# marcin119a/vae-los-angeles

Hardware: AMD Instinct MI355X
Metric: training samples/sec, MultiModalVAE batch 65536 (higher is better)
Workload: dtype bf16

## Files before the change

### include/mmvae_hip.h

```cpp
#ifndef MMVAE_HIP_H
#define MMVAE_HIP_H
#include <stdint.h>

#ifdef __cplusplus
extern "C" {
#endif

#define MMVAE_OK 0
#define MMVAE_ERR_ARG (-1)
#define MMVAE_ERR_DTYPE (-2)

enum { MMVAE_F32 = 0, MMVAE_BF16 = 1 };
enum { MMVAE_PREC_F32 = 0, MMVAE_PREC_BF16 = 1 };
enum { MMVAE_PRO_NONE = 0, MMVAE_PRO_BN_RELU_DROP = 1, MMVAE_PRO_BN_BWD_APPLY = 2 };
enum { MMVAE_EPI_STORE = 0, MMVAE_EPI_RELU_MASK = 1, MMVAE_EPI_BN_BWD = 2, MMVAE_EPI_LOSS_MSE = 3, MMVAE_EPI_LOSS_BCE_LOGIT = 4 };
enum { MMVAE_ACT_NONE = 0, MMVAE_ACT_RELU = 1, MMVAE_ACT_SIGMOID = 2 };

#define MMVAE_TILE 128

int mmvae_abi_version(void);
int mmvae_set_tuning(int32_t key, int32_t value);

typedef struct {
    const float* src; void* dst;
// ... 101 lines not shown
    const void* w; int64_t ldw; const float* bias;
} mmvae_latent_enc;
typedef struct {
    int32_t prec, B, L, n_mod;
    mmvae_latent_enc enc_a, enc_b;
    const float* table; const int64_t* site; int32_t S;
    const float* eps;
    float* mu; float* logvar;
    void* z; int64_t ldz;
    const void* w_stem; int64_t ldw_stem; const float* bias_stem; int32_t N_stem;
    void* h0; int64_t ldh0;
} mmvae_latent_fwd_args;
int mmvae_latent_fwd(const mmvae_latent_fwd_args* args, void* stream);

typedef struct {
    int32_t prec, B, S, L, hidden;
    const void* h0; int64_t ldh0;
    const void* w; int64_t ldw; const void* wt; int64_t ldwt; const float* bias;
    const int64_t* site; const float* class_weights;
    const float* mu; const float* logvar;
    float beta, gamma; const float* beta_gamma_dev;
    double* sums;
    float* g_c; int64_t ld_gc;
    void* d0; int64_t ldd0;
    float* g_mu; float* g_lv;
} mmvae_class_tail_args;
int mmvae_class_tail(const mmvae_class_tail_args* args, void* stream);
int mmvae_class_tail_fits(int32_t prec, int32_t S, int32_t hidden, int32_t L, int64_t ldh0, int64_t ldd0);

typedef struct {
// ... 99 lines not shown
```

### vae-los-angeles_amd/csrc/common.h

```cpp
#pragma once
#include <hip/hip_runtime.h>
#include <stdint.h>
#include "mmvae_hip.h"

namespace mm {

typedef __bf16 bf16;
typedef __attribute__((ext_vector_type(8))) __bf16 bf16x8;
typedef __attribute__((ext_vector_type(4))) __bf16 bf16x4;
typedef __attribute__((ext_vector_type(2))) __bf16 bf16x2;
typedef __attribute__((ext_vector_type(4))) float f32x4;
typedef __attribute__((ext_vector_type(2))) float f32x2;
typedef __attribute__((ext_vector_type(4))) short s16x4;

constexpr int WAVE = 64;
constexpr int TILE = 128;
constexpr int NTHREADS = 256;
constexpr int ROW_BYTES = 128;
constexpr int NUM_CU = 256;

template <typename CT> struct Mma;

template <> struct Mma<bf16> {
    static constexpr int EPC = 8;
// ... 127 lines not shown
#endif


struct Tuning {
    int nt_wide_min_m = NUM_CU * 128;
    int nt2_on = 1;
    long split_bytes = 1L << 32;
    long block_bytes = 1L << 31;
    int tn_wide_on = 1;
    int bnbwd_stream = 1;
    int relu_stream = 1;
    int ntp_on = 1;
    int ntp_min_m = 16384;
    int latent_on = 1;
    int class_tail_on = 1;
};
inline Tuning g_tuning;

constexpr int NOT_TAKEN = 1 << 30;

template <auto Kernel, typename... Args>
inline int launch_lds(dim3 grid, dim3 block, int lds, hipStream_t st, const Args&... args) {
    static bool attr_done = false;
    if (!attr_done) {
        hipError_t e = hipFuncSetAttribute((const void*)Kernel, hipFuncAttributeMaxDynamicSharedMemorySize, lds);
        if (e != hipSuccess) return (int)e;
        attr_done = true;
    }
    hipLaunchKernelGGL(Kernel, grid, block, lds, st, args...);
    return (int)hipGetLastError();
// ... 49 lines not shown
```

### vae-los-angeles_amd/csrc/elementwise.hip

```cpp
#include <vector>
#include "common.h"
#include "mmvae_hip.h"
#include "fuse_math.h"
#include "loss_terms.h"

namespace mm {

__global__ __launch_bounds__(256) void prep_weights_kernel(const mmvae_prep_item* __restrict__ items) {
    const mmvae_prep_item it = items[blockIdx.y];
    __shared__ float tile[32][33];
    const int tx = threadIdx.x & 31, ty = threadIdx.x >> 5;
    const int tiles_c = (it.dst_cols + 31) / 32, tiles_r = (it.dst_rows + 31) / 32;
    auto put = [&](int r, int c, float v) {
        if (it.dst_dtype == MMVAE_BF16) ((bf16*)it.dst)[(long)r * it.dst_ld + c] = (bf16)v;
        else ((float*)it.dst)[(long)r * it.dst_ld + c] = v;
    };
    for (int t = blockIdx.x; t < tiles_r * tiles_c; t += gridDim.x) {
        const int tr = t / tiles_c, tc = t - tr * tiles_c;
        if (it.transpose) {
#pragma unroll
            for (int k = 0; k < 4; ++k) {
                const int sr = tc * 32 + ty + 8 * k, sc = tr * 32 + tx;
                tile[ty + 8 * k][tx] = (sr < it.src_rows && sc < it.src_cols) ? it.src[(long)sr * it.src_ld + sc] : 0.f;
            }
// ... 227 lines not shown
            const long i = min(i0 + (long)u * blockDim.x, iend - 1);
            const int b = (int)(i / a.L), l = (int)(i - (long)b * a.L);
            bb[u] = b; ll[u] = l;
            dz[u] = a.dz[(long)b * a.lddz + l];
            if (a.dz2) dz[u] += a.dz2[(long)b * a.lddz + l];
            if (a.dz3) dz[u] += a.dz3[(long)b * a.lddz + l];
            gm[u] = a.g_mu ? a.g_mu[i] : 0.f; gl[u] = a.g_lv ? a.g_lv[i] : 0.f;
            ep[u] = a.eps[i]; lv[u] = a.logvar[i];
            sidx[u] = a.d_table ? a.site[b] : 0;
            if (sidx[u] < 0 || sidx[u] >= a.S) sidx[u] = -1;
        }
#pragma unroll
        for (int u = 0; u < U; ++u) {
            if (i0 + (long)u * blockDim.x >= iend) break;
            const int b = bb[u], l = ll[u];
            float dmu = gm[u] + dz[u];
            float dlv = gl[u] + dz[u] * ep[u] * expf(0.5f * lv[u]) * 0.5f;
            if (a.n_mod > 1) { dmu *= inv_n; dlv *= inv_n; }
            a.d_heads[(long)b * a.ld_heads + l] = dmu;
            a.d_heads[(long)b * a.ld_heads + a.L + l] = dlv;
            if (a.d_heads_lp) {
                bf16* lp = (bf16*)a.d_heads_lp + (long)b * a.ld_heads_lp;
                lp[l] = (bf16)dmu; lp[a.L + l] = (bf16)dlv;
                if (l == 0) for (int e = 2 * a.L; e < a.ld_heads_lp; ++e) lp[e] = (bf16)0.f;
            }
            if (a.d_table && sidx[u] >= 0) {
                const long sx = sidx[u];
                if (use_lds) { atomicAdd(&sT[sx * L2 + l], dmu); atomicAdd(&sT[sx * L2 + a.L + l], dlv); }
                else { unsafeAtomicAdd(&dtab[sx * L2 + l], dmu); unsafeAtomicAdd(&dtab[sx * L2 + a.L + l], dlv); }
            }
        }
    }
    if (use_lds && a.d_table) {
// ... 750 lines not shown
```

### vae-los-angeles_amd/csrc/fuse_math.h

```cpp
#pragma once
#include "common.h"

namespace mm {

__device__ __forceinline__ float fuse_reparam_elem(float& mu, float& lv, int n_mod, float inv_n, float eps) {
    if (n_mod > 1) { mu *= inv_n; lv *= inv_n; }
    return mu + eps * expf(0.5f * lv);
}

}
```

### vae-los-angeles_amd/csrc/gemm_nt.hip

```cpp
#include "common.h"
#include "mmvae_hip.h"
#include "gemm_src.h"
#include "gemm_nt_epi.h"
#include "gemm_nt2.h"

namespace mm {

STAMP_BUFFER(nt)

__device__ __forceinline__ int swz(int row, int chunk) { return row * ROW_BYTES + ((chunk ^ (row & 7)) << 4); }

template <int WN> struct NtLds {
    static constexpr int BUF = (TILE + 64 * WN) * ROW_BYTES;
    static constexpr int STAGE = 2 * BUF;
    static constexpr int ECOL = STAGE + 4096 + 4 * 64 * WN * 4;
    static constexpr int TOTAL = ECOL + 8 * 64 * WN * 4;
};

template <typename CT, typename Src, typename Epi, int WN>
__global__ __launch_bounds__(128 * WN, 2)
void gemm_nt_kernel(Src src, const CT* __restrict__ W, long ldw, int M, int N, int K, int gx, int gy, Epi epi)
{
    constexpr int EPC = Mma<CT>::EPC;
    constexpr int BK = ROW_BYTES / (int)sizeof(CT);
// ... 293 lines not shown
    switch (key) {
    case 0: t.nt_wide_min_m = value; return 0;
    case 2: t.nt2_on = value; return 0;
    case 3:
        if (value != 0 && (value < 17 || value > 32)) return MMVAE_ERR_ARG;
        t.split_bytes = value ? 1L << value : mm::Tuning{}.split_bytes;
        t.block_bytes = t.split_bytes / 2;
        return 0;
    case 4: t.tn_wide_on = value; return 0;
    case 6: t.bnbwd_stream = value; return 0;
    case 7: t.relu_stream = value; return 0;
    case 8: t.ntp_on = value; return 0;
    case 9: t.ntp_min_m = value; return 0;
    case 10: t.latent_on = value; return 0;
    case 12: t.class_tail_on = value; return 0;
    }
    return MMVAE_ERR_ARG;
}

extern "C" int mmvae_gemm_nt(const mmvae_gemm_nt_args* a, void* stream) {
    if (!a || !a->a || !a->w || (!a->c && !(a->epilogue == MMVAE_EPI_BN_BWD && a->bn_phase == 0))) return MMVAE_ERR_ARG;
    if (a->M <= 0 || a->N <= 0 || a->K <= 0) return MMVAE_ERR_ARG;
    if (a->ldw % 64 || ((uintptr_t)a->w & 15)) return MMVAE_ERR_ARG;
    const long lim = 1L << 32;
    if (((long)a->N + 256) * a->ldw * 4 >= lim) return MMVAE_ERR_ARG;
    const long a_row = (long)a->lda * (a->a_dtype == MMVAE_BF16 ? 2 : 4);
    long row_bytes = a_row > (long)a->ld_pro_mask ? a_row : (long)a->ld_pro_mask;
    if (!mm::bn_fin_ok(a)) return MMVAE_ERR_ARG;
    if (mm::needs_row_blocks(a->M, row_bytes)) {
        if (a->pro_finalize || a->pro_out) return MMVAE_ERR_ARG;
// ... 23 lines not shown
```

### vae-los-angeles_amd/csrc/gemm_nt2.h

```cpp
#pragma once
#include "common.h"
#include "gemm_nt_epi.h"

namespace mm {

template <int WN> struct Nt2Lds {
    static constexpr int A_BYTES = TILE * ROW_BYTES;
    static constexpr int W_BYTES = 64 * WN * ROW_BYTES;
    static constexpr int SLOT = A_BYTES + W_BYTES;
    static constexpr int RING = 2 * SLOT;
    static constexpr int RED = RING;
    static constexpr int ECOL = RED + 4 * 64 * WN * 4;
    static constexpr int TOTAL = ECOL + 8 * 64 * WN * 4;
};

STAMP_BUFFER(nt2)

typedef __attribute__((address_space(3))) void lds_void;
typedef __attribute__((address_space(1))) const void gbl_void;

template <typename Epi, int WN>
__device__ __forceinline__ void nt2_loss_epilogue(unsigned char* smem, const float* ecol, float* red, f32x4 (&acc)[4][4], const Epi& epi,
                                                  int row0, int col0, int M, int N, int tid, int lane, int wr, int wc)
{
// ... 147 lines not shown
    __syncthreads();
    const int ccols = (int)min((long)((N + 7) & ~7), epi.ldc);
    const unsigned char* src = smem + r0 * 512 + ((c ^ (r0 & 7)) << 4);
    float sc[4], sh[4], mu[4], rs[4], s1[4] = {0.f, 0.f, 0.f, 0.f}, s2[4] = {0.f, 0.f, 0.f, 0.f};
#pragma unroll
    for (int e = 0; e < 4; ++e) { sc[e] = ecol[4 * c + e]; sh[e] = ecol[BN + 4 * c + e]; mu[e] = ecol[2 * BN + 4 * c + e]; rs[e] = ecol[3 * BN + 4 * c + e]; }
#pragma unroll
    for (int i = 0; i < 16; ++i) {
        const int grow = row0 + r0 + 8 * i;
        const f32x4 z = *(const f32x4*)(src + i * 8 * 512);
        bf16x4 o;
#pragma unroll
        for (int e = 0; e < 4; ++e) {
            const bool ok = grow < M && colg + e < N;
            const float y = (float)yv[i][e];
            const float keep = ((mv[i] >> (8 * e)) & 0xffu) ? epi.inv_keep : 0.f;
            const float d = (ok && y * sc[e] + sh[e] > 0.f) ? z[e] * (has_mask ? keep : 1.f) : 0.f;
            const float xh = (y - mu[e]) * rs[e];
            s1[e] += d; s2[e] += d * xh;
            o[e] = (bf16)d;
        }
        if (grow < M && colg < ccols) *(bf16x4*)(C + (long)grow * epi.ldc + colg) = o;
    }
    __syncthreads();
    float* part = (float*)smem;
#pragma unroll
    for (int e = 0; e < 4; ++e) { part[(r0 * 2 + 0) * BN + 4 * c + e] = s1[e]; part[(r0 * 2 + 1) * BN + 4 * c + e] = s2[e]; }
    __syncthreads();
    if (tid < 2 * BN) {
        const int which = tid >> 7, col = tid & (BN - 1);
        float v = 0.f;
#pragma unroll
        for (int g = 0; g < 8; ++g) v += part[(g * 2 + which) * BN + col];
// ... 145 lines not shown
```

### vae-los-angeles_amd/mmvae/_lib.py

```python
import ctypes as C
import os

_HERE = os.path.dirname(os.path.abspath(__file__))
LIB_PATH = os.environ.get("MMVAE_LIB_PATH") or os.path.join(_HERE, "libmmvae_hip.so")
ABI_VERSION = 20

F32, BF16 = 0, 1
PREC_F32, PREC_BF16 = 0, 1
PRO_NONE, PRO_BN_RELU_DROP, PRO_BN_BWD_APPLY = 0, 1, 2
TABLE_COPIES = 8
EPI_STORE, EPI_RELU_MASK, EPI_BN_BWD, EPI_LOSS_MSE, EPI_LOSS_BCE_LOGIT = 0, 1, 2, 3, 4
ACT_NONE, ACT_RELU, ACT_SIGMOID = 0, 1, 2
TILE = 128
TN_GROUP_MAX = 8
KNN_MAXK = 64
SIL_MAXC = 64
PCA_MAXK = 64
CTR_COPIES = 16384

i32, i64, f32, vp = C.c_int32, C.c_int64, C.c_float, C.c_void_p


class PrepItem(C.Structure):
    _fields_ = [("src", vp), ("dst", vp), ("src_rows", i32), ("src_cols", i32), ("src_ld", i64),
# ... 55 lines not shown

class LatentEnc(C.Structure):
    _fields_ = [("y", vp), ("ldy", i64), ("K", i32), ("scale", vp), ("shift", vp),
                ("mask", vp), ("ld_mask", i64), ("inv_keep", f32), ("finalize", vp),
                ("w", vp), ("ldw", i64), ("bias", vp)]


class LatentFwdArgs(C.Structure):
    _fields_ = [("prec", i32), ("B", i32), ("L", i32), ("n_mod", i32),
                ("enc_a", LatentEnc), ("enc_b", LatentEnc),
                ("table", vp), ("site", vp), ("S", i32),
                ("eps", vp), ("mu", vp), ("logvar", vp),
                ("z", vp), ("ldz", i64),
                ("w_stem", vp), ("ldw_stem", i64), ("bias_stem", vp), ("N_stem", i32),
                ("h0", vp), ("ldh0", i64)]


class ClassTailArgs(C.Structure):
    _fields_ = [("prec", i32), ("B", i32), ("S", i32), ("L", i32), ("hidden", i32),
                ("h0", vp), ("ldh0", i64),
                ("w", vp), ("ldw", i64), ("wt", vp), ("ldwt", i64), ("bias", vp),
                ("site", vp), ("class_weights", vp),
                ("mu", vp), ("logvar", vp),
                ("beta", f32), ("gamma", f32), ("beta_gamma_dev", vp),
                ("sums", vp),
                ("g_c", vp), ("ld_gc", i64),
                ("d0", vp), ("ldd0", i64),
                ("g_mu", vp), ("g_lv", vp)]


# ... 62 lines not shown
    "mmvae_set_tuning": [i32, i32],
    "mmvae_prep_weights": [vp, i32, vp],
    "mmvae_gemm_nt": [C.POINTER(GemmNtArgs), vp],
    "mmvae_gemm_tn": [C.POINTER(GemmTnArgs), vp],
    "mmvae_gemm_tn_group": [vp, i32, vp],
    "mmvae_bn_finalize": [C.POINTER(BnFinalizeArgs), vp],
    "mmvae_bn_eval_coeffs": [i32, vp, vp, vp, vp, f32, vp, vp, vp, vp, vp],
    "mmvae_bn_bwd_finalize": [C.POINTER(BnBwdFinalizeArgs), vp],
    "mmvae_bn_bwd_apply": [i32, i32, i32, vp, i64, vp, i64, vp, vp, vp, vp],
    "mmvae_bn_bwd_finalize_apply": [i32, i32, i32, vp, i64, vp, i64, vp, vp, vp, vp, vp, vp, vp, i32, vp],
    "mmvae_embed_table_fwd": [i32, i32, i32, vp, vp, vp, vp, vp, vp, vp],
    "mmvae_embed_table_bwd": [i32, i32, i32, vp, vp, vp, vp, i32, vp, vp, vp, vp, vp, vp],
    "mmvae_fuse_reparam_fwd": [C.POINTER(FuseFwdArgs), vp],
    "mmvae_fuse_reparam_bwd": [C.POINTER(FuseBwdArgs), vp],
    "mmvae_latent_fwd": [C.POINTER(LatentFwdArgs), vp],
    "mmvae_class_tail": [C.POINTER(ClassTailArgs), vp],
    "mmvae_class_tail_fits": [i32, i32, i32, i32, i64, i64],
    "mmvae_vae_loss": [C.POINTER(LossArgs), vp],
    "mmvae_loss_finalize": [vp, f32, f32, vp, vp, vp],
    "mmvae_recon_metrics": [C.POINTER(MetricsArgs), vp],
    "mmvae_knn_search": [C.POINTER(KnnArgs), vp],
    "mmvae_knn_work_bytes": [i32, i32, i32, C.POINTER(i64)],
    "mmvae_knn_splits": [i32, i32, C.POINTER(i32), C.POINTER(i32)],
    "mmvae_knn_mean_rows": [vp, i64, vp, i32, i64, vp, i64, i32, i32, i32, i32, vp],
    "mmvae_silhouette_samples": [C.POINTER(SilhouetteArgs), vp],
    "mmvae_silhouette_work_bytes": [i32, i32, i32, C.POINTER(i64)],
    "mmvae_silhouette_splits": [i32, i32, i32, C.POINTER(i32)],
    "mmvae_pca_scatter": [C.POINTER(PcaScatterArgs), vp],
    "mmvae_pca_scatter_splits": [i32, i32, i32, C.POINTER(i32)],
    "mmvae_pca_scatter_work_bytes": [i32, i32, i32, C.POINTER(i64)],
# ... 51 lines not shown
```

### vae-los-angeles_amd/mmvae/engine.py

```python
import os
from dataclasses import dataclass
from typing import NamedTuple, Optional

import torch

from . import ops
from . import _lib as L_
from .ops import (PREC_BF16, PREC_F32, ACT_NONE, ACT_RELU, ACT_SIGMOID, EPI_RELU_MASK, EPI_BN_BWD, DROP_P,
                  ceil_to, act_dtype, Prologue, BnBwdEpilogue, BnBwdFinalize, BnBwdApply)

_PRECISIONS = {"bf16": PREC_BF16, "fp32": PREC_F32, "f32": PREC_F32}
_default_precision = _PRECISIONS[os.environ.get("MMVAE_PRECISION", "bf16").lower()]
_TINY_DW_MAX = 16384


def set_default_precision(name):
    global _default_precision
    _default_precision = _PRECISIONS[name.lower()]


def default_precision():
    return _default_precision


# ... 254 lines not shown
            else:
                ops.gemm_nt(prec, h, pl.w, N, K, y, bias=pl.bias, prologue=pro, tag=f"{self.name}.L{len(layers)}.fwd")
                ops.bn_eval_coeffs(bn.weight, bn.bias, bn.running_mean, bn.running_var, st.scale, st.shift, bn.eps, st.mean, st.rstd)
                new_pro = Prologue(st.scale, st.shift, None, 1.0)
            layers.append(LayerSave(h, pro, y, st, new_pro) if h_act is None else LayerSave(h_act, None, y, st, new_pro))
            h, pro = y, new_pro
        owed = ops.LatentEncoder(h, pro, fin, self.pl_heads)
        return (self.run_heads(prec, owed) if heads else owed), layers

    def run_heads(self, prec, owed):
        heads = torch.empty(owed.y.shape[0], 2 * self.latent, dtype=torch.float32, device=owed.y.device)
        self._consume(prec, owed.y, owed.prologue, owed.fin, 2 * self.latent, self.pl_heads.K, heads, self.pl_heads.bias, self.pl_heads.w,
                      f"{self.name}.heads.fwd")
        return heads

    def backward(self, prec, layers, d_heads, grads, tn=ops.gemm_tn, stats_bufs=None, train=True, d_heads_lp=None):
        B, dev = d_heads.shape[0], d_heads.device
        adt = act_dtype(prec)
        L2 = 2 * self.latent
        Kl = self.pl_heads.K
        gw = grads[self.fc_mu.weight]
        gb = grads[self.fc_mu.bias]
        tn(prec, d_heads, layers[-1].y, _span(gw, L2 * Kl).view(L2, Kl), _span(gb, L2), L2, Kl, q_prologue=layers[-1].y_prologue, tag=f"{self.name}.heads.dW")
        src, src_wt, src_n, src_k = (d_heads_lp if d_heads_lp is not None else d_heads), self.pl_heads.wt, Kl, L2
        for i in reversed(range(len(self.linears))):
            lin, bn, pl = self.linears[i], self.bns[i], self.pl[i]
            sv = layers[i]
            y = sv.y
            st = sv.bn
            N, K = pl.N, pl.K
            bnargs = BnBwdEpilogue(st.scale, st.shift, st.mean, st.rstd, sv.y_prologue.mask, sv.y_prologue.inv_keep)
            stats = stats_bufs[i] if stats_bufs is not None else torch.zeros(2, N, dtype=torch.float64, device=dev)
            coef = torch.empty(3, N, dtype=torch.float32, device=dev)
            d = torch.empty(B, ceil_to(N, 8), dtype=adt, device=dev)
            ops.gemm_nt(prec, src, src_wt, src_n, src_k, d, epilogue=EPI_BN_BWD, h=y, bn=bnargs, bn_phase=2, stats=stats, tag=f"{self.name}.L{i}.dX")
            fin = BnBwdFinalize(stats, bn.weight, grads[bn.weight], grads[bn.bias], not train)
            if i == 0 and K <= 4096:
                if prec == PREC_BF16 and B >= 8192 and N >= 128 and K >= 256:
                    try:
                        tn(prec, d, sv.q, grads[lin.weight], grads[lin.bias], N, K, q_prologue=sv.q_prologue,
                           p_prologue=BnBwdApply(y, st.mean, st.rstd, fin=fin), tag=f"{self.name}.L{i}.dW")
                        continue
                    except L_.MMVAEArgError:
                        pass
                ops.bn_bwd_finalize(B, N, stats, bn.weight, st.rstd, grads[bn.weight], grads[bn.bias], coef, eval_mode=not train)
                tn(prec, d, sv.q, grads[lin.weight], grads[lin.bias], N, K, q_prologue=sv.q_prologue,
                   p_prologue=BnBwdApply(y, st.mean, st.rstd, coef), tag=f"{self.name}.L{i}.dW")
                continue
            try:
                ops.bn_bwd_finalize_apply(d, y, B, N, st.mean, st.rstd, *fin)
# ... 260 lines not shown
            else:
                o, acts = dec.forward(prec, z, first=firsts[i])
            outs[i] = o
            state.dec[i] = (acts, o.detach())
        return outs, mu, logvar, state

    def _class_tail_index(self, prec, H0, want, site):
        if self.dec_stem is None or site is None or H0 is None:
            return None
        for i, dec in enumerate(self.decoders):
            if want[i] is None and isinstance(dec, DecoderMLP) and len(dec.pl) == 2 and not dec.final_sigmoid \
                    and ops.class_tail_fits(prec, dec.pl[1].N, dec.pl[1].K, self.latent, H0.stride(0), H0.stride(0)):
                return i
        return None

    def backward(self, state, g_outs, g_logit_flags, g_mu, g_lv):
        with ops.pinned_stream():
            return self._backward(state, g_outs, g_logit_flags, g_mu, g_lv)

    def _backward(self, state, g_outs, g_logit_flags, g_mu, g_lv):
        prec, B = state.prec, state.B
        site = state.site
        dev = state.eps.device
        Ld = self.latent
        zeros, state.zeros = state.zeros, None
        if zeros is None:
            zeros = self.zero_pack(dev, state.enc_a is not None, state.enc_b is not None, site is not None, fwd=False, bwd=True)
        flat = zeros.arena
        grads = carve_arena(flat, self.param_list())
        n_a = len(state.enc_a) if state.enc_a is not None else 0
# ... 20 lines not shown
        if stem is not None:
            D0 = tail.d0 if tail is not None else torch.empty(B, stem.N, dtype=act_dtype(prec), device=dev)
        for i, (dec, (acts, out), g, is_logit) in enumerate(zip(self.decoders, state.dec, g_outs, g_logit_flags)):
            n0 = dec.linears[0].out_features if stem is not None else 0
            if g is None:
                off += n0
                continue
            dx_done = tail.d0_slice if (tail is not None and tail.index == i and tail.done) else None
            if stem is not None:
                dec.backward(prec, acts, out, g, is_logit, None, grads, tn, d0_out=D0[:, off:off + n0], dx_done=dx_done)
                off += n0
                continue
            dz = torch.empty(B, Ld, dtype=torch.float32, device=dev)
            dec.backward(prec, acts, out, g, is_logit, dz, grads, tn, dx_done=dx_done)
            dzs.append(dz)
        if stem is not None:
            dz = torch.empty(B, Ld, dtype=torch.float32, device=dev)
            ops.gemm_nt(prec, D0, stem.wt, stem.K, stem.N, dz, tag="Decoders.L0.dX")
            dzs.append(dz)
        if not dzs:
            dzs.append(torch.zeros(B, Ld, dtype=torch.float32, device=dev))
        if self.grad_sync is not None:
            self.grad_sync.early(flat, self.early_cut())
        d_heads = torch.empty(B, 2 * Ld, dtype=torch.float32, device=dev)
        d_heads_lp = torch.empty(B, ceil_to(2 * Ld, 8), dtype=torch.bfloat16, device=dev) if prec == PREC_BF16 else None
        ops.fuse_reparam_bwd(B, Ld, state.n_mod, g_mu, g_lv, dzs, state.eps, state.logvar, d_heads, zeros.d_table, site, d_heads_lp=d_heads_lp)
        if state.enc_a is not None:
            self.enc_a.backward(prec, state.enc_a, d_heads, grads, tn, zeros.bwd_stats[:n_a], train=state.train, d_heads_lp=d_heads_lp)
        if state.enc_b is not None:
            self.enc_b.backward(prec, state.enc_b, d_heads, grads, tn, zeros.bwd_stats[n_a:], train=state.train, d_heads_lp=d_heads_lp)
        if site is not None:
            self.enc_c.backward(zeros.d_table, grads)
        flush_tiny("tiny_dW.heads")
        if self.grad_sync is not None:
            self.grad_sync.final(flat)
        return flat, grads
```

### vae-los-angeles_amd/mmvae/ops.py

```python
import ctypes as C
from collections import namedtuple

import torch

from . import _lib as L
from ._lib import (F32, BF16, PREC_F32, PREC_BF16, PRO_NONE, PRO_BN_RELU_DROP, PRO_BN_BWD_APPLY, EPI_STORE, EPI_RELU_MASK,
                   EPI_BN_BWD, EPI_LOSS_MSE, EPI_LOSS_BCE_LOGIT, ACT_NONE, ACT_RELU, ACT_SIGMOID, TILE)

DROP_P = 0.1
BN_EPS, BN_MOMENTUM = 1e-5, 0.1


class KernelProbe:

    def __init__(self, only=None):
        self.records = {}
        self.only = only

    def wants(self, tag):
        return tag is not None and (self.only is None or tag in self.only)

    def begin(self):
        ev = torch.cuda.Event(enable_timing=True)
        ev.record(torch.cuda.current_stream())
# ... 418 lines not shown
    a.z, a.ldz = z.data_ptr(), _ld(z)
    a.w_stem, a.ldw_stem, a.bias_stem, a.N_stem = stem.w.data_ptr(), stem.w.stride(0), _p(stem.bias), stem.N
    a.h0, a.ldh0 = h0.data_ptr(), _ld(h0)
    return a, B * nbytes


def latent_fwd(prec, B, Ld, enc_a, enc_b, table, site, eps, mu, logvar, z, stem, h0):
    for t in (eps, mu, logvar):
        if tuple(t.shape) != (B, Ld) or not t.is_contiguous():
            raise ValueError(f"latent_fwd: eps / mu / logvar must be contiguous ({B}, {Ld}), got {tuple(t.shape)} / {t.stride()}")
    a, nbytes = latent_fwd_args(prec, B, Ld, enc_a, enc_b, table, site, eps, mu, logvar, z, stem, h0)
    with stream_span("latent.fwd", nbytes):
        L.check(L.load().mmvae_latent_fwd(C.byref(a), _stream()), "mmvae_latent_fwd")


def fuse_reparam_bwd(B, Ld, n_mod, g_mu, g_lv, dzs, eps, logvar, d_heads, d_table, site, d_heads_lp=None):
    dzs = list(dzs) + [None] * (3 - len(dzs))
    copies = d_table.shape[0] if (d_table is not None and d_table.dim() == 3) else 1
    a = L.FuseBwdArgs(B, Ld, n_mod, _p(g_mu), _p(g_lv), dzs[0].data_ptr(), _p(dzs[1]), _p(dzs[2]), _ld(dzs[0]), eps.data_ptr(), logvar.data_ptr(),
                      d_heads.data_ptr(), _ld(d_heads), _p(d_table), _p(site), d_table.shape[-2] if d_table is not None else 0,
                      _p(d_heads_lp), _ld(d_heads_lp) if d_heads_lp is not None else 0, copies)
    n_dz = sum(1 for d in dzs if d is not None)
    with stream_span("fuse_reparam_bwd", B * Ld * 4 * (n_dz + (g_mu is not None) + (g_lv is not None) + 2 + 2)):
        L.check(L.load().mmvae_fuse_reparam_bwd(C.byref(a), _stream()), "mmvae_fuse_reparam_bwd")


def loss_workspace(device):
    buf = torch.zeros(5 * 8 + 5 * 4 + 4, dtype=torch.uint8, device=device)
    return buf[:40].view(torch.float64), buf[40:60].view(torch.float32)

# ... 355 lines not shown
```

Before: 53.27 million.

## Fuse stem dX, reparam backward and encoder head BN-backward into one latent kernel

```diff
diff --git a/include/mmvae_hip.h b/include/mmvae_hip.h
--- a/include/mmvae_hip.h
+++ b/include/mmvae_hip.h
@@ -139,6 +139,26 @@
 int mmvae_latent_fwd(const mmvae_latent_fwd_args* args, void* stream);
 
 typedef struct {
+    const void* y; int64_t ldy; int32_t K;
+    const float* scale; const float* shift; const float* mean; const float* rstd;
+    const uint8_t* mask; int64_t ld_mask; float inv_keep;
+    const void* wt; int64_t ldwt;
+    void* d; int64_t ldd;
+    double* stat1; double* stat2;
+} mmvae_latent_bwd_enc;
+typedef struct {
+    int32_t prec, B, L, n_mod;
+    const void* d0; int64_t ldd0; int32_t N_stem;
+    const void* wt_stem; int64_t ldwt_stem;
+    const float* g_mu; const float* g_lv; const float* eps; const float* logvar;
+    float* d_heads;
+    float* d_table; const int64_t* site; int32_t S; int32_t table_copies;
+    mmvae_latent_bwd_enc enc_a, enc_b;
+} mmvae_latent_bwd_args;
+int mmvae_latent_bwd(const mmvae_latent_bwd_args* args, void* stream);
+int mmvae_latent_bwd_fp32_rows(int32_t B);
+
+typedef struct {
     int32_t prec, B, S, L, hidden;
     const void* h0; int64_t ldh0;
     const void* w; int64_t ldw; const void* wt; int64_t ldwt; const float* bias;
diff --git a/vae-los-angeles_amd/csrc/common.h b/vae-los-angeles_amd/csrc/common.h
--- a/vae-los-angeles_amd/csrc/common.h
+++ b/vae-los-angeles_amd/csrc/common.h
@@ -165,6 +165,7 @@
     int ntp_min_m = 16384;
     int latent_on = 1;
     int class_tail_on = 1;
+    int latent_bwd_on = 1;
 };
 inline Tuning g_tuning;
 
diff --git a/vae-los-angeles_amd/csrc/elementwise.hip b/vae-los-angeles_amd/csrc/elementwise.hip
--- a/vae-los-angeles_amd/csrc/elementwise.hip
+++ b/vae-los-angeles_amd/csrc/elementwise.hip
@@ -265,9 +265,8 @@
         for (int u = 0; u < U; ++u) {
             if (i0 + (long)u * blockDim.x >= iend) break;
             const int b = bb[u], l = ll[u];
-            float dmu = gm[u] + dz[u];
-            float dlv = gl[u] + dz[u] * ep[u] * expf(0.5f * lv[u]) * 0.5f;
-            if (a.n_mod > 1) { dmu *= inv_n; dlv *= inv_n; }
+            float dmu, dlv;
+            fuse_reparam_bwd_elem(gm[u], gl[u], dz[u], ep[u], lv[u], a.n_mod, inv_n, dmu, dlv);
             a.d_heads[(long)b * a.ld_heads + l] = dmu;
             a.d_heads[(long)b * a.ld_heads + a.L + l] = dlv;
             if (a.d_heads_lp) {
diff --git a/vae-los-angeles_amd/csrc/fuse_math.h b/vae-los-angeles_amd/csrc/fuse_math.h
--- a/vae-los-angeles_amd/csrc/fuse_math.h
+++ b/vae-los-angeles_amd/csrc/fuse_math.h
@@ -8,4 +8,19 @@
     return mu + eps * expf(0.5f * lv);
 }
 
+__device__ __forceinline__ void fuse_reparam_bwd_elem(float g_mu, float g_lv, float dz, float eps, float lv, int n_mod, float inv_n,
+                                                      float& dmu, float& dlv) {
+    dmu = g_mu + dz;
+    dlv = g_lv + dz * eps * expf(0.5f * lv) * 0.5f;
+    if (n_mod > 1) { dmu *= inv_n; dlv *= inv_n; }
 }
+
+__device__ __forceinline__ float bn_relu_drop_bwd_elem(float z, float y, bool ok, bool has_mask, unsigned keep_byte, float inv_keep,
+                                                       float sc, float sh, float mu, float rs, float& xh) {
+    const float keep = keep_byte ? inv_keep : 0.f;
+    const float d = (ok && y * sc + sh > 0.f) ? z * (has_mask ? keep : 1.f) : 0.f;
+    xh = (y - mu) * rs;
+    return d;
+}
+
+}
diff --git a/vae-los-angeles_amd/csrc/gemm_nt.hip b/vae-los-angeles_amd/csrc/gemm_nt.hip
--- a/vae-los-angeles_amd/csrc/gemm_nt.hip
+++ b/vae-los-angeles_amd/csrc/gemm_nt.hip
@@ -331,6 +331,7 @@
     case 9: t.ntp_min_m = value; return 0;
     case 10: t.latent_on = value; return 0;
     case 12: t.class_tail_on = value; return 0;
+    case 13: t.latent_bwd_on = value; return 0;
     }
     return MMVAE_ERR_ARG;
 }
diff --git a/vae-los-angeles_amd/csrc/gemm_nt2.h b/vae-los-angeles_amd/csrc/gemm_nt2.h
--- a/vae-los-angeles_amd/csrc/gemm_nt2.h
+++ b/vae-los-angeles_amd/csrc/gemm_nt2.h
@@ -1,6 +1,7 @@
 #pragma once
 #include "common.h"
 #include "gemm_nt_epi.h"
+#include "fuse_math.h"
 
 namespace mm {
 
@@ -185,9 +186,8 @@
         for (int e = 0; e < 4; ++e) {
             const bool ok = grow < M && colg + e < N;
             const float y = (float)yv[i][e];
-            const float keep = ((mv[i] >> (8 * e)) & 0xffu) ? epi.inv_keep : 0.f;
-            const float d = (ok && y * sc[e] + sh[e] > 0.f) ? z[e] * (has_mask ? keep : 1.f) : 0.f;
-            const float xh = (y - mu[e]) * rs[e];
+            float xh;
+            const float d = bn_relu_drop_bwd_elem(z[e], y, ok, has_mask, (mv[i] >> (8 * e)) & 0xffu, epi.inv_keep, sc[e], sh[e], mu[e], rs[e], xh);
             s1[e] += d; s2[e] += d * xh;
             o[e] = (bf16)d;
         }
diff --git a/vae-los-angeles_amd/csrc/latent_bwd.hip b/vae-los-angeles_amd/csrc/latent_bwd.hip
--- /dev/null
+++ b/vae-los-angeles_amd/csrc/latent_bwd.hip
@@ -0,0 +1,312 @@
+#include "common.h"
+#include "mmvae_hip.h"
+#include "gemm_src.h"
+#include "fuse_math.h"
+#include "wave_slab.h"
+
+namespace mm {
+
+constexpr int LATB_WAVES = 8, LATB_THREADS = 64 * LATB_WAVES;
+constexpr int LATB_NKS = 14;
+constexpr int LATB_NB = 4;
+constexpr int LATB_FU = 6;
+constexpr int LATB_HC = 12;
+constexpr int LATB_MAXTAB = 1024;
+constexpr int LATB_SROW = LATB_NKS * 64 + 16;
+constexpr int LATB_HROW = 128 + 16;
+constexpr int LATB_DZLD = 36;
+constexpr int LATB_OFF_WH = 32 * LATB_SROW;
+constexpr int LATB_OFF_TAB = LATB_OFF_WH + 2 * 256 * LATB_HROW;
+constexpr int LATB_OFF_DT = LATB_OFF_TAB + 2 * 4 * 256 * 4;
+constexpr int LATB_OFF_SCR = LATB_OFF_DT + LATB_MAXTAB * 4;
+constexpr int LATB_SCR_F = 16 * 48 * 4;
+constexpr int LATB_SCR = LATB_SCR_F + 16 * LATB_HROW;
+constexpr int LATB_LDS = LATB_OFF_SCR + LATB_WAVES * LATB_SCR;
+static_assert(16 * LATB_DZLD * 4 <= LATB_SCR_F, "the dz image lies in the d_heads image");
+static_assert(LATB_WAVES * 2 * 2 * 256 * 4 <= 2 * 256 * LATB_HROW, "the final sums lie in the heads operand");
+static_assert(LATB_LDS <= 160 * 1024, "LDS of one CU");
+
+struct LatbEnc {
+    const bf16* y; long ldy; const uint8_t* mask; long ldm; float inv_keep;
+    const float* tab[4];
+    const bf16* wt; long ldwt;
+    bf16* d; long ldd; double* stat1; double* stat2;
+    int nb;
+};
+struct LatbArgs {
+    LatbEnc e[2];
+    int B, L, n_mod, S, copies, nks, nslabs;
+    const bf16* d0; long ldd0; const bf16* wts; long ldwts;
+    const float* g_mu; const float* g_lv; const float* eps; const float* logvar;
+    float* d_heads; float* d_table; const long long* site;
+};
+
+__device__ __forceinline__ void rows_sum2_into(float u, float v, float sel, float& t1, float& t2) {
+    asm volatile("s_nop 1\n\t"
+                 "v_add_f32_dpp %0, %0, %0 row_ror:8 row_mask:0xf bank_mask:0xf\n\tv_add_f32_dpp %1, %1, %1 row_ror:8 row_mask:0xf bank_mask:0xf\n\ts_nop 1\n\t"
+                 "v_add_f32_dpp %0, %0, %0 row_ror:4 row_mask:0xf bank_mask:0xf\n\tv_add_f32_dpp %1, %1, %1 row_ror:4 row_mask:0xf bank_mask:0xf\n\ts_nop 1\n\t"
+                 "v_add_f32_dpp %0, %0, %0 row_ror:2 row_mask:0xf bank_mask:0xf\n\tv_add_f32_dpp %1, %1, %1 row_ror:2 row_mask:0xf bank_mask:0xf\n\ts_nop 1\n\t"
+                 "v_add_f32_dpp %0, %0, %0 row_ror:1 row_mask:0xf bank_mask:0xf\n\tv_add_f32_dpp %1, %1, %1 row_ror:1 row_mask:0xf bank_mask:0xf\n\t"
+                 "v_fmac_f32 %2, %0, %4\n\tv_fmac_f32 %3, %1, %4"
+                 : "+v"(u), "+v"(v), "+v"(t1), "+v"(t2) : "v"(sel));
+}
+
+__global__ __launch_bounds__(LATB_THREADS) void latent_bwd_kernel(const LatbArgs a) {
+    extern __shared__ __attribute__((aligned(16))) unsigned char smem[];
+    const int tid = threadIdx.x, lane = tid & 63, wid = tid >> 6;
+    const int li = lane & 15, lg = lane >> 4;
+    float* const stab = (float*)(smem + LATB_OFF_TAB);
+    float* const sdt = (float*)(smem + LATB_OFF_DT);
+    unsigned char* const scr = smem + LATB_OFF_SCR + wid * LATB_SCR;
+    float* const sf = (float*)scr;
+    unsigned char* const sa = scr + LATB_SCR_F;
+    const int L = a.L, L2 = 2 * a.L;
+    const float inv_n = 1.f / (float)a.n_mod;
+    const int total = a.B * L, total2 = a.B * L2;
+
+
+    bf16x8 rd0[LATB_NKS];
+    float gm_r[LATB_FU], gl_r[LATB_FU], ep_r[LATB_FU], lv_r[LATB_FU];
+    long long site_r = 0;
+    auto fetch_d0 = [&](int slab) __attribute__((always_inline)) {
+        const unsigned ro = (unsigned)min(slab * 16 + li, a.B - 1) * (unsigned)a.ldd0 + (unsigned)(8 * lg);
+#pragma unroll
+        for (int j = 0; j < LATB_NKS; ++j) rd0[j] = *(const bf16x8*)(a.d0 + (ro + 32u * (unsigned)min(j, a.nks - 1)));
+    };
+    const float* const gmp = a.g_mu ? a.g_mu : a.eps;
+    const float* const glp = a.g_lv ? a.g_lv : a.eps;
+    auto fetch_fu = [&](int slab) __attribute__((always_inline)) {
+#pragma unroll
+        for (int i = 0; i < LATB_FU; ++i) {
+            const int idx = min(slab * 16 * L + lane + 64 * i, total - 1);
+            ep_r[i] = a.eps[idx]; lv_r[i] = a.logvar[idx]; gm_r[i] = gmp[idx]; gl_r[i] = glp[idx];
+        }
+        if (a.d_table) site_r = a.site[min(slab * 16 + li, a.B - 1)];
+    };
+
+    const int nw = gridDim.x * LATB_WAVES;
+    int slab = blockIdx.x * LATB_WAVES + wid;
+    const bool any = slab < a.nslabs;
+    if (any) { fetch_d0(slab); fetch_fu(slab); }
+
+    stage_rows<LATB_THREADS>(smem, LATB_SROW, a.wts, a.ldwts, 32, a.nks * 4, tid, [](int x) { return x; });
+#pragma unroll
+    for (int e = 0; e < 2; ++e) {
+        if (a.e[e].nb == 0) continue;
+        stage_rows<LATB_THREADS>(smem + LATB_OFF_WH + e * 256 * LATB_HROW, LATB_HROW, a.e[e].wt, a.e[e].ldwt, 64 * a.e[e].nb, 8, tid,
+                                 [](int x) { return (x & ~63) + EpiCols<true>::wrow(x & 63); });
+#pragma unroll
+        for (int w = 0; w < 4; ++w)
+            for (int col = tid; col < 64 * a.e[e].nb; col += LATB_THREADS) stab[(e * 4 + w) * 256 + col] = a.e[e].tab[w][col];
+    }
+    if (a.d_table) for (int i = tid; i < a.S * L2; i += LATB_THREADS) sdt[i] = 0.f;
+    for (int i = lane; i < 16 * LATB_HROW / 16; i += 64) ((uint4*)sa)[i] = uint4{0u, 0u, 0u, 0u};
+    __syncthreads();
+
+    float s1[2][LATB_NB] = {}, s2[2][LATB_NB] = {};
+    if (any) for (;;) {
+        int lane_v = lane;
+        asm volatile("" : "+v"(lane_v));
+        const int li = lane_v & 15, lg = lane_v >> 4;
+        int fr[LATB_FU], fl[LATB_FU];
+#pragma unroll
+        for (int i = 0; i < LATB_FU; ++i) { const int x = lane_v + 64 * i; fr[i] = x / L; fl[i] = x - fr[i] * L; }
+        const bool lowl = li < 8;
+        {
+            f32x4 dz[2] = {f32x4{0.f, 0.f, 0.f, 0.f}, f32x4{0.f, 0.f, 0.f, 0.f}};
+#pragma unroll
+            for (int j = 0; j < LATB_NKS; ++j) {
+                if (j < a.nks) {
+#pragma unroll
+                    for (int n = 0; n < 2; ++n) {
+                        const bf16x8 wf = *(const bf16x8*)(smem + (16 * n + li) * LATB_SROW + (4 * j + lg) * 16);
+                        Mma<bf16>::mma(dz[n], wf, rd0[j]);
+                    }
+                }
+            }
+#pragma unroll
+            for (int n = 0; n < 2; ++n) *(f32x4*)(sf + li * LATB_DZLD + 16 * n + 4 * lg) = dz[n];
+        }
+        bf16x8 ry[2][LATB_NB][2];
+        uint2 rm[2][LATB_NB][2];
+        auto fetch_y = [&](int e) __attribute__((always_inline)) {
+            const unsigned row = (unsigned)min(slab * 16 + li, a.B - 1);
+#pragma unroll
+            for (int p = 0; p < LATB_NB; ++p) {
+                if (p >= a.e[e].nb) continue;
+                const unsigned col = (unsigned)(64 * p + 8 * lg);
+                const bf16* yp = a.e[e].y + (row * (unsigned)a.e[e].ldy + col);
+                ry[e][p][0] = *(const bf16x8*)yp; ry[e][p][1] = *(const bf16x8*)(yp + 32);
+                rm[e][p][0] = rm[e][p][1] = uint2{0u, 0u};
+                if (a.e[e].mask) {
+                    const uint8_t* mp = a.e[e].mask + (row * (unsigned)a.e[e].ldm + col);
+                    rm[e][p][0] = *(const uint2*)mp; rm[e][p][1] = *(const uint2*)(mp + 32);
+                }
+            }
+        };
+        fetch_y(0); fetch_y(1);
+        wave_lds_sync();
+
+        float dzv[LATB_FU], gm[LATB_FU], gl[LATB_FU], ep[LATB_FU], lv[LATB_FU];
+        long long st[LATB_FU];
+#pragma unroll
+        for (int i = 0; i < LATB_FU; ++i) {
+            const int rr = min(fr[i], 15);
+            dzv[i] = sf[rr * LATB_DZLD + fl[i]];
+            gm[i] = a.g_mu ? gm_r[i] : 0.f; gl[i] = a.g_lv ? gl_r[i] : 0.f; ep[i] = ep_r[i]; lv[i] = lv_r[i];
+            const unsigned lo = (unsigned)__builtin_amdgcn_ds_bpermute(4 * rr, (int)(unsigned)site_r);
+            const unsigned hi = (unsigned)__builtin_amdgcn_ds_bpermute(4 * rr, (int)(unsigned)((unsigned long long)site_r >> 32));
+            st[i] = (long long)(((unsigned long long)hi << 32) | lo);
+        }
+        wave_lds_sync();
+#pragma unroll
+        for (int i = 0; i < LATB_FU; ++i) {
+            if (lane_v + 64 * i >= 16 * L) break;
+            const int r = fr[i], l = fl[i];
+            float dmu, dlv;
+            fuse_reparam_bwd_elem(gm[i], gl[i], dzv[i], ep[i], lv[i], a.n_mod, inv_n, dmu, dlv);
+            const bool real = slab * 16 * L + lane_v + 64 * i < total;
+            if (!real) { dmu = 0.f; dlv = 0.f; }
+            sf[r * L2 + l] = dmu; sf[r * L2 + L + l] = dlv;
+            ((bf16*)sa)[r * (LATB_HROW / 2) + l] = (bf16)dmu; ((bf16*)sa)[r * (LATB_HROW / 2) + L + l] = (bf16)dlv;
+            if (a.d_table && real && st[i] >= 0 && st[i] < a.S) {
+                const int sx = (int)st[i];
+                atomicAdd(&sdt[sx * L2 + l], dmu); atomicAdd(&sdt[sx * L2 + L + l], dlv);
+            }
+        }
+        wave_lds_sync();
+#pragma unroll
+        for (int i = 0; i < LATB_HC; ++i) {
+            const int x = lane_v + 64 * i;
+            if (x < 16 * L2 && slab * 16 * L2 + x < total2) a.d_heads[slab * 16 * L2 + x] = sf[x];
+        }
+
+        const bf16x8 af0 = *(const bf16x8*)(sa + li * LATB_HROW + lg * 16), af1 = *(const bf16x8*)(sa + li * LATB_HROW + 64 + lg * 16);
+        const bool rowok = slab * 16 + li < a.B;
+        const int rbase = slab * 16 + (li & 7);
+        const bool ok0 = rbase < a.B, ok1 = rbase + 8 < a.B;
+#pragma unroll
+        for (int e = 0; e < 2; ++e) {
+            if (a.e[e].nb == 0) continue;
+            const bool has_mask = a.e[e].mask != nullptr;
+            const float inv_keep = a.e[e].inv_keep;
+            bf16* const crow = line_col(a.e[e].d + (long)rbase * a.e[e].ldd, li, lg);
+#pragma unroll
+            for (int p = 0; p < LATB_NB; ++p) {
+                if (p >= a.e[e].nb) break;
+                f32x4 acc[4];
+#pragma unroll
+                for (int q = 0; q < 4; ++q) {
+                    const unsigned char* wp = smem + LATB_OFF_WH + (e * 256 + 64 * p + 16 * q + li) * LATB_HROW + lg * 16;
+                    acc[q] = f32x4{0.f, 0.f, 0.f, 0.f};
+                    Mma<bf16>::mma(acc[q], *(const bf16x8*)wp, af0);
+                    Mma<bf16>::mma(acc[q], *(const bf16x8*)(wp + 64), af1);
+                }
+                uint32_t pk[2][4];
+                float t1 = 0.f, t2 = 0.f;
+#pragma unroll
+                for (int h = 0; h < 2; ++h) {
+                    const float* tp = stab + e * 4 * 256 + 64 * p + 32 * h + 8 * lg;
+                    const bf16x8 yv = ry[e][p][h];
+                    const uint2 mv = rm[e][p][h];
+                    float d[8];
+#pragma unroll
+                    for (int i = 0; i < 8; ++i) {
+                        const unsigned kb = ((i < 4 ? mv.x : mv.y) >> (8 * (i & 3))) & 0xffu;
+                        float xh;
+                        d[i] = bn_relu_drop_bwd_elem(acc[2 * h + (i >> 2)][i & 3], (float)yv[i], rowok, has_mask, kb, inv_keep,
+                                                     tp[i], tp[256 + i], tp[512 + i], tp[768 + i], xh);
+                        rows_sum2_into(d[i], d[i] * xh, li == 8 * h + i ? 1.f : 0.f, t1, t2);
+                    }
+#pragma unroll
+                    for (int qd = 0; qd < 4; ++qd) {
+                        const bf16x2 t = {(bf16)d[2 * qd], (bf16)d[2 * qd + 1]};
+                        pk[h][qd] = __builtin_bit_cast(uint32_t, t);
+                    }
+                }
+                s1[e][p] += t1; s2[e][p] += t2;
+                SWAP_HALVES(pk, lowl, st0, st1);
+                if (ok0) *(uint4*)(crow + 64 * p) = uint4{st0[0], st0[1], st0[2], st0[3]};
+                if (ok1) *(uint4*)(crow + 8 * a.e[e].ldd + 64 * p) = uint4{st1[0], st1[1], st1[2], st1[3]};
+            }
+        }
+        slab += nw;
+        if (slab >= a.nslabs) break;
+        fetch_d0(slab); fetch_fu(slab);
+        wave_lds_sync();
+    }
+
+    __syncthreads();
+    float* const part = (float*)(smem + LATB_OFF_WH);
+#pragma unroll
+    for (int e = 0; e < 2; ++e)
+#pragma unroll
+        for (int p = 0; p < LATB_NB; ++p) {
+            if (p >= a.e[e].nb) break;
+            const int col = 64 * p + 32 * (li >> 3) + 8 * lg + (li & 7);
+            part[((wid * 2 + e) * 2 + 0) * 256 + col] = s1[e][p]; part[((wid * 2 + e) * 2 + 1) * 256 + col] = s2[e][p];
+        }
+    __syncthreads();
+#pragma unroll
+    for (int e = 0; e < 2; ++e) {
+        const int which = tid >> 8, col = tid & 255;
+        if (col >= 64 * a.e[e].nb) continue;
+        float v = 0.f;
+#pragma unroll
+        for (int w = 0; w < LATB_WAVES; ++w) v += part[((w * 2 + e) * 2 + which) * 256 + col];
+        if (v != 0.f) unsafeAtomicAdd((which ? a.e[e].stat2 : a.e[e].stat1) + col, (double)v);
+    }
+    if (a.d_table) {
+        float* const dtab = a.d_table + (long)(blockIdx.x % a.copies) * a.S * L2;
+        for (int i = tid; i < a.S * L2; i += LATB_THREADS) if (sdt[i] != 0.f) unsafeAtomicAdd(&dtab[i], sdt[i]);
+    }
+}
+
+static int latb_enc(const mmvae_latent_bwd_enc& e, int B, LatbEnc& o) {
+    o = LatbEnc{};
+    if (!e.y) return 0;
+    if (e.K < 64 || e.K % 64 || e.K > 64 * LATB_NB || e.ldy % 8 || e.ldy < e.K || ((uintptr_t)e.y & 15)) return MMVAE_ERR_ARG;
+    if (!e.scale || !e.shift || !e.mean || !e.rstd || !e.stat1 || !e.stat2) return MMVAE_ERR_ARG;
+    if (e.mask && (e.ld_mask % 8 || e.ld_mask < e.K || ((uintptr_t)e.mask & 7))) return MMVAE_ERR_ARG;
+    if (!e.wt || e.ldwt % 8 || e.ldwt < 64 || ((uintptr_t)e.wt & 15)) return MMVAE_ERR_ARG;
+    if (!e.d || e.ldd % 64 || e.ldd < e.K || ((uintptr_t)e.d & 127)) return MMVAE_ERR_ARG;
+    const long lim = 1L << 32;
+    if ((long)B * e.ldy * 2 >= lim || (long)B * e.ldd * 2 >= lim || (e.mask && (long)B * e.ld_mask >= lim)) return MMVAE_ERR_ARG;
+    o.y = (const bf16*)e.y; o.ldy = e.ldy; o.mask = e.mask; o.ldm = e.ld_mask; o.inv_keep = e.inv_keep;
+    o.tab[0] = e.scale; o.tab[1] = e.shift; o.tab[2] = e.mean; o.tab[3] = e.rstd;
+    o.wt = (const bf16*)e.wt; o.ldwt = e.ldwt; o.d = (bf16*)e.d; o.ldd = e.ldd; o.stat1 = e.stat1; o.stat2 = e.stat2;
+    o.nb = e.K / 64;
+    return 0;
+}
+
+}
+
+extern "C" int mmvae_latent_bwd_fp32_rows(int32_t B) {
+    using namespace mm;
+    if (B <= 0) return MMVAE_ERR_ARG;
+    const int nslabs = (B + 15) / 16, per_round = LATB_WAVES * persistent_grid(nslabs, LATB_WAVES);
+    return LATB_WAVES * 16 * ((nslabs + per_round - 1) / per_round);
+}
+
+extern "C" int mmvae_latent_bwd(const mmvae_latent_bwd_args* a, void* stream) {
+    using namespace mm;
+    if (!a || !g_tuning.latent_bwd_on) return MMVAE_ERR_ARG;
+    if (a->prec != MMVAE_PREC_BF16) return MMVAE_ERR_DTYPE;
+    if (a->B <= 0 || a->L <= 0 || a->L > 24 || (long)a->B * 2 * a->L >= (1L << 31)) return MMVAE_ERR_ARG;
+    if (!a->d0 || !a->wt_stem || !a->eps || !a->logvar || !a->d_heads) return MMVAE_ERR_ARG;
+    const int present = (a->enc_a.y != nullptr) + (a->enc_b.y != nullptr) + (a->d_table != nullptr);
+    if (present == 0 || present != a->n_mod) return MMVAE_ERR_ARG;
+    if (a->d_table && (!a->site || a->S <= 0 || (long)a->S * 2 * a->L > LATB_MAXTAB || a->table_copies < 0)) return MMVAE_ERR_ARG;
+    if (a->N_stem < 64 || a->N_stem % 64 || a->N_stem > 32 * LATB_NKS) return MMVAE_ERR_ARG;
+    if (a->ldd0 % 64 || a->ldd0 < a->N_stem || ((uintptr_t)a->d0 & 127) || (long)a->B * a->ldd0 * 2 >= (1L << 32)) return MMVAE_ERR_ARG;
+    if (a->ldwt_stem % 8 || a->ldwt_stem < a->N_stem || ((uintptr_t)a->wt_stem & 15)) return MMVAE_ERR_ARG;
+    LatbArgs k{};
+    { const int rc = latb_enc(a->enc_a, a->B, k.e[0]); if (rc) return rc; }
+    { const int rc = latb_enc(a->enc_b, a->B, k.e[1]); if (rc) return rc; }
+    k.B = a->B; k.L = a->L; k.n_mod = a->n_mod; k.S = a->S; k.copies = a->table_copies > 0 ? a->table_copies : 1;
+    k.nks = a->N_stem / 32; k.nslabs = (a->B + 15) / 16;
+    k.d0 = (const bf16*)a->d0; k.ldd0 = a->ldd0; k.wts = (const bf16*)a->wt_stem; k.ldwts = a->ldwt_stem;
+    k.g_mu = a->g_mu; k.g_lv = a->g_lv; k.eps = a->eps; k.logvar = a->logvar;
+    k.d_heads = a->d_heads; k.d_table = a->d_table; k.site = (const long long*)a->site;
+    return launch_lds<latent_bwd_kernel>(dim3(persistent_grid(k.nslabs, LATB_WAVES)), dim3(LATB_THREADS), LATB_LDS, (hipStream_t)stream, k);
+}
diff --git a/vae-los-angeles_amd/mmvae/_lib.py b/vae-los-angeles_amd/mmvae/_lib.py
--- a/vae-los-angeles_amd/mmvae/_lib.py
+++ b/vae-los-angeles_amd/mmvae/_lib.py
@@ -93,6 +93,22 @@
                 ("z", vp), ("ldz", i64),
                 ("w_stem", vp), ("ldw_stem", i64), ("bias_stem", vp), ("N_stem", i32),
                 ("h0", vp), ("ldh0", i64)]
+
+
+class LatentBwdEnc(C.Structure):
+    _fields_ = [("y", vp), ("ldy", i64), ("K", i32), ("scale", vp), ("shift", vp), ("mean", vp), ("rstd", vp),
+                ("mask", vp), ("ld_mask", i64), ("inv_keep", f32),
+                ("wt", vp), ("ldwt", i64), ("d", vp), ("ldd", i64), ("stat1", vp), ("stat2", vp)]
+
+
+class LatentBwdArgs(C.Structure):
+    _fields_ = [("prec", i32), ("B", i32), ("L", i32), ("n_mod", i32),
+                ("d0", vp), ("ldd0", i64), ("N_stem", i32),
+                ("wt_stem", vp), ("ldwt_stem", i64),
+                ("g_mu", vp), ("g_lv", vp), ("eps", vp), ("logvar", vp),
+                ("d_heads", vp),
+                ("d_table", vp), ("site", vp), ("S", i32), ("table_copies", i32),
+                ("enc_a", LatentBwdEnc), ("enc_b", LatentBwdEnc)]
 
 
 class ClassTailArgs(C.Structure):
@@ -185,6 +201,8 @@
     "mmvae_fuse_reparam_fwd": [C.POINTER(FuseFwdArgs), vp],
     "mmvae_fuse_reparam_bwd": [C.POINTER(FuseBwdArgs), vp],
     "mmvae_latent_fwd": [C.POINTER(LatentFwdArgs), vp],
+    "mmvae_latent_bwd": [C.POINTER(LatentBwdArgs), vp],
+    "mmvae_latent_bwd_fp32_rows": [i32],
     "mmvae_class_tail": [C.POINTER(ClassTailArgs), vp],
     "mmvae_class_tail_fits": [i32, i32, i32, i32, i64, i64],
     "mmvae_vae_loss": [C.POINTER(LossArgs), vp],
diff --git a/vae-los-angeles_amd/mmvae/engine.py b/vae-los-angeles_amd/mmvae/engine.py
--- a/vae-los-angeles_amd/mmvae/engine.py
+++ b/vae-los-angeles_amd/mmvae/engine.py
@@ -292,7 +292,13 @@
                       f"{self.name}.heads.fwd")
         return heads
 
-    def backward(self, prec, layers, d_heads, grads, tn=ops.gemm_tn, stats_bufs=None, train=True, d_heads_lp=None):
+    def latent_bwd_operand(self, layers, stats_bufs):
+        sv, i = layers[-1], len(self.linears) - 1
+        d = torch.empty(sv.y.shape[0], ceil_to(self.pl[i].N, 8), dtype=torch.bfloat16, device=sv.y.device)
+        bn = BnBwdEpilogue(sv.bn.scale, sv.bn.shift, sv.bn.mean, sv.bn.rstd, sv.y_prologue.mask, sv.y_prologue.inv_keep)
+        return ops.LatentBwdEncoder(sv.y, bn, self.pl_heads, d, stats_bufs[i])
+
+    def backward(self, prec, layers, d_heads, grads, tn=ops.gemm_tn, stats_bufs=None, train=True, d_heads_lp=None, d_last=None):
         B, dev = d_heads.shape[0], d_heads.device
         adt = act_dtype(prec)
         L2 = 2 * self.latent
@@ -310,8 +316,11 @@
             bnargs = BnBwdEpilogue(st.scale, st.shift, st.mean, st.rstd, sv.y_prologue.mask, sv.y_prologue.inv_keep)
             stats = stats_bufs[i] if stats_bufs is not None else torch.zeros(2, N, dtype=torch.float64, device=dev)
             coef = torch.empty(3, N, dtype=torch.float32, device=dev)
-            d = torch.empty(B, ceil_to(N, 8), dtype=adt, device=dev)
-            ops.gemm_nt(prec, src, src_wt, src_n, src_k, d, epilogue=EPI_BN_BWD, h=y, bn=bnargs, bn_phase=2, stats=stats, tag=f"{self.name}.L{i}.dX")
+            if d_last is not None and i == len(self.linears) - 1:
+                d = d_last
+            else:
+                d = torch.empty(B, ceil_to(N, 8), dtype=adt, device=dev)
+                ops.gemm_nt(prec, src, src_wt, src_n, src_k, d, epilogue=EPI_BN_BWD, h=y, bn=bnargs, bn_phase=2, stats=stats, tag=f"{self.name}.L{i}.dX")
             fin = BnBwdFinalize(stats, bn.weight, grads[bn.weight], grads[bn.bias], not train)
             if i == 0 and K <= 4096:
                 if prec == PREC_BF16 and B >= 8192 and N >= 128 and K >= 256:
@@ -602,6 +611,12 @@
                 return i
         return None
 
+    @staticmethod
+    def _stem_dx(prec, D0, stem, B, Ld, dev):
+        dz = torch.empty(B, Ld, dtype=torch.float32, device=dev)
+        ops.gemm_nt(prec, D0, stem.wt, stem.K, stem.N, dz, tag="Decoders.L0.dX")
+        return dz
+
     def backward(self, state, g_outs, g_logit_flags, g_mu, g_lv):
         with ops.pinned_stream():
             return self._backward(state, g_outs, g_logit_flags, g_mu, g_lv)
@@ -652,21 +667,31 @@
             dz = torch.empty(B, Ld, dtype=torch.float32, device=dev)
             dec.backward(prec, acts, out, g, is_logit, dz, grads, tn, dx_done=dx_done)
             dzs.append(dz)
-        if stem is not None:
-            dz = torch.empty(B, Ld, dtype=torch.float32, device=dev)
-            ops.gemm_nt(prec, D0, stem.wt, stem.K, stem.N, dz, tag="Decoders.L0.dX")
-            dzs.append(dz)
-        if not dzs:
+        try_fused = stem is not None and prec == PREC_BF16 and state.train
+        if stem is not None and not try_fused:
+            dzs.append(self._stem_dx(prec, D0, stem, B, Ld, dev))
+        if not dzs and not try_fused:
             dzs.append(torch.zeros(B, Ld, dtype=torch.float32, device=dev))
         if self.grad_sync is not None:
             self.grad_sync.early(flat, self.early_cut())
         d_heads = torch.empty(B, 2 * Ld, dtype=torch.float32, device=dev)
-        d_heads_lp = torch.empty(B, ceil_to(2 * Ld, 8), dtype=torch.bfloat16, device=dev) if prec == PREC_BF16 else None
-        ops.fuse_reparam_bwd(B, Ld, state.n_mod, g_mu, g_lv, dzs, state.eps, state.logvar, d_heads, zeros.d_table, site, d_heads_lp=d_heads_lp)
+        d_heads_lp, d_a, d_b = None, None, None
+        if try_fused:
+            op_a = self.enc_a.latent_bwd_operand(state.enc_a, zeros.bwd_stats[:n_a]) if state.enc_a is not None else None
+            op_b = self.enc_b.latent_bwd_operand(state.enc_b, zeros.bwd_stats[n_a:]) if state.enc_b is not None else None
+            try:
+                ops.latent_bwd(prec, B, Ld, D0, stem, g_mu, g_lv, state.eps, state.logvar, d_heads, zeros.d_table, site, op_a, op_b)
+                d_a, d_b = (op_a.d if op_a is not None else None), (op_b.d if op_b is not None else None)
+            except L_.MMVAEArgError:
+                try_fused = False
+                dzs.append(self._stem_dx(prec, D0, stem, B, Ld, dev))
+        if not try_fused:
+            d_heads_lp = torch.empty(B, ceil_to(2 * Ld, 8), dtype=torch.bfloat16, device=dev) if prec == PREC_BF16 else None
+            ops.fuse_reparam_bwd(B, Ld, state.n_mod, g_mu, g_lv, dzs, state.eps, state.logvar, d_heads, zeros.d_table, site, d_heads_lp=d_heads_lp)
         if state.enc_a is not None:
-            self.enc_a.backward(prec, state.enc_a, d_heads, grads, tn, zeros.bwd_stats[:n_a], train=state.train, d_heads_lp=d_heads_lp)
+            self.enc_a.backward(prec, state.enc_a, d_heads, grads, tn, zeros.bwd_stats[:n_a], train=state.train, d_heads_lp=d_heads_lp, d_last=d_a)
         if state.enc_b is not None:
-            self.enc_b.backward(prec, state.enc_b, d_heads, grads, tn, zeros.bwd_stats[n_a:], train=state.train, d_heads_lp=d_heads_lp)
+            self.enc_b.backward(prec, state.enc_b, d_heads, grads, tn, zeros.bwd_stats[n_a:], train=state.train, d_heads_lp=d_heads_lp, d_last=d_b)
         if site is not None:
             self.enc_c.backward(zeros.d_table, grads)
         flush_tiny("tiny_dW.heads")
diff --git a/vae-los-angeles_amd/mmvae/ops.py b/vae-los-angeles_amd/mmvae/ops.py
--- a/vae-los-angeles_amd/mmvae/ops.py
+++ b/vae-los-angeles_amd/mmvae/ops.py
@@ -456,6 +456,54 @@
         L.check(L.load().mmvae_latent_fwd(C.byref(a), _stream()), "mmvae_latent_fwd")
 
 
+LatentBwdEncoder = namedtuple("LatentBwdEncoder", "y bn heads d stats")
+
+
+def latent_bwd_fp32_rows(B):
+    n = L.load().mmvae_latent_bwd_fp32_rows(B)
+    L.check(min(n, 0), "mmvae_latent_bwd_fp32_rows")
+    return n
+
+
+def latent_bwd_args(prec, B, Ld, d0, stem, g_mu, g_lv, eps, logvar, d_heads, d_table, site, enc_a, enc_b):
+    a = L.LatentBwdArgs()
+    a.prec, a.B, a.L = prec, B, Ld
+    a.n_mod = (enc_a is not None) + (enc_b is not None) + (d_table is not None)
+    a.d0, a.ldd0, a.N_stem = _mat(d0, "d0").data_ptr(), _ld(d0), stem.N
+    a.wt_stem, a.ldwt_stem = stem.wt.data_ptr(), stem.wt.stride(0)
+    a.g_mu, a.g_lv, a.eps, a.logvar, a.d_heads = _p(g_mu), _p(g_lv), eps.data_ptr(), logvar.data_ptr(), d_heads.data_ptr()
+    nbytes = d0.element_size() * stem.N + 4 * Ld * (4 + (g_mu is not None) + (g_lv is not None)) + 8 * (d_table is not None)
+    if d_table is not None:
+        a.d_table, a.site, a.S = d_table.data_ptr(), _p(site), d_table.shape[-2]
+        a.table_copies = d_table.shape[0] if d_table.dim() == 3 else 1
+    for e, enc in ((a.enc_a, enc_a), (a.enc_b, enc_b)):
+        if enc is None:
+            continue
+        sc, sh, mean, rstd, mask, inv_keep = enc.bn
+        e.y, e.ldy, e.K = _mat(enc.y, "y").data_ptr(), _ld(enc.y), enc.heads.K
+        e.scale, e.shift, e.mean, e.rstd = sc.data_ptr(), sh.data_ptr(), mean.data_ptr(), rstd.data_ptr()
+        e.mask, e.ld_mask, e.inv_keep = _p(mask), (_ld(mask) if mask is not None else 0), inv_keep
+        e.wt, e.ldwt = enc.heads.wt.data_ptr(), enc.heads.wt.stride(0)
+        e.d, e.ldd = _mat(enc.d, "d").data_ptr(), _ld(enc.d)
+        e.stat1, e.stat2 = enc.stats[0].data_ptr(), enc.stats[1].data_ptr()
+        nbytes += enc.heads.K * (enc.y.element_size() + (mask is not None) + enc.d.element_size())
+    return a, B * nbytes
+
+
+def latent_bwd(prec, B, Ld, d0, stem, g_mu, g_lv, eps, logvar, d_heads, d_table, site, enc_a, enc_b):
+    for t in (g_mu, g_lv, eps, logvar):
+        if t is not None and (tuple(t.shape) != (B, Ld) or not t.is_contiguous() or t.dtype != torch.float32):
+            raise ValueError(f"latent_bwd: g_mu / g_lv / eps / logvar must be contiguous fp32 ({B}, {Ld}), got {tuple(t.shape)} / {t.stride()}")
+    if tuple(d_heads.shape) != (B, 2 * Ld) or not d_heads.is_contiguous() or d_heads.dtype != torch.float32:
+        raise ValueError(f"latent_bwd: d_heads must be contiguous fp32 ({B}, {2 * Ld})")
+    for enc in (enc_a, enc_b):
+        if enc is not None:
+            assert enc.stats.dtype == torch.float64 and enc.stats.shape[0] == 2 and enc.stats.stride(1) == 1
+    a, nbytes = latent_bwd_args(prec, B, Ld, d0, stem, g_mu, g_lv, eps, logvar, d_heads, d_table, site, enc_a, enc_b)
+    with stream_span("Latent.bwd", nbytes):
+        L.check(L.load().mmvae_latent_bwd(C.byref(a), _stream()), "mmvae_latent_bwd")
+
+
 def fuse_reparam_bwd(B, Ld, n_mod, g_mu, g_lv, dzs, eps, logvar, d_heads, d_table, site, d_heads_lp=None):
     dzs = list(dzs) + [None] * (3 - len(dzs))
     copies = d_table.shape[0] if (d_table is not None and d_table.dim() == 3) else 1
```

Result: no change. 52.81 million (-0.9%).
